# NVlabs/few-shot-vid2vid

Hardware: AMD Instinct MI355X
Metric: frames/sec G+D fwd+bwd step, 512x512 fewshot_pose (higher is better)
Workload: dtype f32; 1 GPU; fewshot_pose 512x512, per-GPU batch 2, adaptive_spade+warp_ref+spade_combine, D step + G step (train.py:58-62), Adam included, no VGG / no FlowNet2 / face-D; global_batch=2, parallelism=dp1, launch=hipgraph

## Files before the change

few-shot-vid2vid_amd/conv.py:

```python
import ctypes
import os
import threading

import torch

from . import lib, profile

ACT_NONE, ACT_LRELU, ACT_TANH, ACT_SIGMOID, ACT_RELU, ACT_LRELU01, ACT_DLRELU = (
    lib.ENUMS["FSV_ACT_" + k] for k in ("NONE", "LRELU", "TANH", "SIGMOID", "RELU", "LRELU01", "DLRELU"))

MFMA_F32, MFMA_F16, MFMA_BF16X3 = 0, 1, 2
_MFMA_NAMES = {'': 0, '0': 0, 'f32': 0, 'fp32': 0, '1': 1, 'f16': 1, 'fp16': 1, '2': 2, 'bf16x3': 2}
_mfma_mode = _MFMA_NAMES[os.environ.get('FSV_MFMA_MODE', '').lower()]


def set_mfma_mode(mode):
    global _mfma_mode
    prev = _mfma_mode
    _mfma_mode = _MFMA_NAMES[str(mode).lower()] if not isinstance(mode, int) else int(mode)
    if _mfma_mode not in (0, 1, 2):
        _mfma_mode = prev
        raise ValueError("unknown MFMA operand mode %r" % (mode,))
    return prev

# ... 368 lines not shown
        if ns > 1 and act != ACT_DLRELU:
            split_ws = torch.empty(ns * out.numel(), dtype=torch.float32, device=x.device)
    ws_args = (lib.ptr(split_ws), split_ws.numel() if split_ws is not None else 0)
    if entry == "fsv_conv_gather_fwd_np":
        if up:
            raise ValueError("a folded up-sampling needs the exact-fp32 kernels (conv.up_foldable)")
        args = head + (_np_mode, lib.stream_ptr())
    else:
        args = head + ws_args + (1 if up else 0, lib.stream_ptr())
    if (stats is not None and grp is None and entry == "fsv_conv_gather_fwd" and place is None and not per_sample
            and not accumulate and force_tile < 0 and force_split == 0 and cin % 4 == 0 and stats_enabled()):
        groups = int(stats['groups'])
        part = stats_arena(x.device).take(groups * STATS_SLOTS * cout * 2)
        prezeroed = part is not None
        if part is None:
            part = torch.empty(groups * STATS_SLOTS * cout * 2, dtype=torch.float64, device=x.device)
        produced = ctypes.c_int(0)
        sargs = (lib.ptr(x), lib.ptr(wt), lib.ptr(bias), lib.ptr(res), lib.ptr(out), n, h, w, cin, oh, ow, cout, len(ty),
                 lib.int_array(ty), lib.int_array(tx), sy, sx, ldw, act, float(scale), lib.ptr(wscale), lib.ptr(part), groups,
                 STATS_SLOTS, 1 if prezeroed else 0, ctypes.byref(produced)) + ws_args + (1 if up else 0, lib.stream_ptr())
        label = 'fsv_conv_igemm_kernel'
        if profile.enabled():
            label = profile.conv_label(n * oh * ow, cout, (len(ty) * cin + 31) // 32, 1, True, force_tile, force_split)
        keep = (x, wt, bias, res, out, wscale, part, split_ws)

        def go_stats(sargs=sargs, keep=keep):
            lib.call("fsv_conv_gather_fwd_stats", *sargs)
        with profile.scope(label, 2.0 * n * oh * ow * cout * cin * len(ty), replay=go_stats):
            go_stats()
        if produced.value:
            stats['part'], stats['slots'] = part, STATS_SLOTS
        return out
    if grp is not None and entry == "fsv_conv_gather_fwd" and force_tile < 0 and force_split == 0:
        d = ConvDesc()
        d.inp, d.wt, d.bias, d.res, d.out, d.wscale = (t.data_ptr() if t is not None else None
                                                       for t in (x, wt, bias, res, out, wscale))
        d.N, d.H, d.W, d.Cin, d.OH, d.OW, d.Cout, d.ntaps = n, h, w, cin, oh, ow, cout, len(ty)
        for i, (a, b) in enumerate(zip(ty, tx)):
            d.ty[i], d.tx[i] = a, b
        d.sy, d.sx, d.outH, d.outW, d.osy, d.osx, d.ooy, d.oox, d.ldw = sy, sx, out_h, out_w, osy, osx, ooy, oox, ldw
        d.per_sample, d.act, d.accumulate, d.scale = (1 if per_sample else 0), act, (1 if accumulate else 0), float(scale)
        d.w_bstride, d.b_bstride = w_bs, b_bs
        label = 'fsv_conv_igemm_kernel'
        if profile.enabled():
            label = profile.conv_label(oh * ow if per_sample else n * oh * ow, cout, (len(ty) * cin + 31) // 32,
                                       n if per_sample else 1, cin % 4 == 0, force_tile, force_split)
        grp.convs.append((d, entry, args, label, 2.0 * n * oh * ow * cout * cin * len(ty), (x, wt, bias, res, out, wscale)))
        return out
    if profile.enabled():
        mz = oh * ow if per_sample else n * oh * ow
        label = profile.conv_label(mz, cout, (len(ty) * cin + 31) // 32, n if per_sample else 1, cin % 4 == 0,
                                   force_tile, force_split,
                                   thin=0 if entry.endswith('_np') else _thin_k(cout, cin, len(ty), per_sample, place, accumulate,
                                                                                force_tile, force_split, act))
        if entry.endswith('_np'):
            label = label.replace('fsv_conv_igemm_kernel', 'fsv_np_conv_kernel[%s]' % ('f16' if _np_mode == 1 else 'bf16x3'))
        keep = (x, wt, bias, res, out, wscale, split_ws)

        def go(entry=entry, args=args, keep=keep):
            lib.call(entry, *args)
        with profile.scope(label, 2.0 * n * oh * ow * cout * cin * len(ty), replay=go):
            go()
    else:
        lib.call(entry, *args)
    return out


_tickets = {}
_TICKET_POOL = 1 << 16


def ticket_range(like, n):
    n = (max(int(n), 1) + 63) // 64 * 64
    if n > _TICKET_POOL // 4:
        return None
    ent = _tickets.get(like.device)
    if ent is None:
        from . import streams
        ent = _tickets[like.device] = [streams.shared(lambda: torch.zeros(_TICKET_POOL, dtype=torch.int32, device=like.device)), 0]
    pool, cur = ent
    if cur + n > _TICKET_POOL:
        cur = 0
    ent[1] = (cur + n) % _TICKET_POOL
    return ctypes.c_void_p(pool.data_ptr() + 4 * cur)


def ordered_split():
    return os.environ.get('FSV_ORDERED_SPLIT', '1') == '1'


def _thin_k(cout, cin, ntaps, per_sample, place, accumulate, force_tile, force_split, act):
    q = cin >> 2
    ok = (cout <= 4 and cin % 4 == 0 and cin <= 256 and q & (q - 1) == 0 and ntaps * cin <= 1152 and not per_sample and
          place is None and not accumulate and force_tile < 0 and force_split <= 0 and act != ACT_DLRELU)
    return ntaps * cin if ok else 0


def conv_forward(x, wt_f, ldw, cout, geom, bias=None, res=None, act=ACT_NONE, scale=1.0, per_sample=False,
                 force_tile=-1, force_split=0, wscale=None, stats=None, up=False):
    n, cin, h, w = x.shape
    oh, ow = geom.out_hw(2 * h, 2 * w) if up else geom.out_hw(h, w)
    return gather_gemm(x, wt_f, ldw, cout, oh, ow, geom.ty, geom.tx, geom.stride, geom.stride, bias=bias, res=res,
                       act=act, scale=scale, per_sample=per_sample, force_tile=force_tile, force_split=force_split,
                       wscale=wscale, stats=stats, up=up)


def planned(mz, cout, nchunks, nsamp, force_tile=-1, force_split=0):
    tile, nsplit = ctypes.c_int(0), ctypes.c_int(1)
    lib.call("fsv_conv_plan", mz, cout, nchunks, nsamp, force_tile, force_split, ctypes.byref(tile), ctypes.byref(nsplit))
    return tile.value, nsplit.value


def _planned_split(mz, cout, nchunks, nsamp):
    return planned(mz, cout, nchunks, nsamp)[1]


_plan_log = None


def start_plan_log():
    global _plan_log
    _plan_log = []


def stop_plan_log():
    global _plan_log
    log, _plan_log = _plan_log, None
    return log or []


def conv_dgrad(dout, w, geom, in_hw, scale=None, per_sample=False, cached=None, cin=None, out_half=False):
    dout = to_nhwc(dout)
    n, cout, oh, ow = dout.shape
    cin = w.shape[-3] if cin is None else cin
    h, wd = in_hw
    s = geom.stride
    if dout.dtype == torch.float16:
        from . import hconv
        layouts = []
        for k, c in enumerate(geom.dgrad_classes):
            if not c['khs']:
                layouts.append(None)
            elif cached is not None:
                layouts.append(half_twin(cached[k][0]))
            else:
                wt_k, _, _ = prep_weight(w, 1, geom, c['khs'], c['kws'], None)
                layouts.append(half_twin(wt_k))
        return hconv.conv_dgrad_h(dout, layouts, geom, in_hw, cin, scale=scale, per_sample=per_sample, out_half=out_half)
# ... 22 lines not shown
            mz = sh * sw if per_sample else n * sh * sw
            if _planned_split(mz, cin, (len(c['khs']) * cout + 31) // 32, n if per_sample else 1) > 1:
                plain = False
                break
    dx = empty_nhwc(n, cin, h, wd, dout) if plain else zeros_nhwc(n, cin, h, wd, dout)
    with launch_group(grouped):
        for k, (c, (sub_h, sub_w)) in enumerate(zip(geom.dgrad_classes, subs)):
            if sub_h <= 0 or sub_w <= 0 or not c['khs']:
                continue
            wt, ldw, ws = layout(k, c)
            gather_gemm(dout, wt, ldw, cin, sub_h, sub_w, c['ty'], c['tx'], 1, 1, per_sample=per_sample, out=dx,
                        place=(h, wd, s, s, c['py'], c['px']), accumulate=not plain, wscale=ws)
    return dx


def conv_wgrad(x, dout, geom, w_shape, per_sample=False, scale=None, force_split=0, out=None, raw=False, arena=None,
               force_tile=0, up=False):
    x = to_nhwc(x)
    dout = to_nhwc(dout)
    n, cin, h, w = x.shape
    if up:
        if x.dtype != torch.float32 or dout.dtype != torch.float32 or per_sample or narrow_staging_mode():
            raise ValueError("a folded up-sampling needs the exact-fp32 kernels (conv.up_foldable)")
        h, w = 2 * h, 2 * w
    _, cout, oh, ow = dout.shape
    if x.dtype == torch.float16 or dout.dtype == torch.float16:
        from . import hconv
        if hconv.wgrad_eligible(cin, cout, oh, ow) and force_tile == 0:
            dwt = hconv.conv_wgrad_h(hconv.to_half_nhwc(x), hconv.to_half_nhwc(dout), geom, per_sample=per_sample,
                                     force_split=force_split, arena=arena if raw else None)
            if raw:
                return dwt
            return unprep_weight_grad(dwt, tuple(w_shape), geom, scale, out)
        x, dout = hconv.cast(x, torch.float32), hconv.cast(dout, torch.float32)
    kpad = _ceil(geom.ntaps * cin, 32)
    ldw = _ceil(cout, 32)
    nb = n if per_sample else 1
    dwt = arena.take(kpad * ldw) if (arena is not None and raw and not per_sample) else None
    prezeroed = dwt is not None
    if dwt is None:
        dwt = torch.empty((nb, kpad, ldw), dtype=torch.float32, device=x.device)
    lib.check_device(x, dout)
    kdim, vec4 = geom.ntaps * cin, cin % 4 == 0
    bn = 32 if cout <= 32 else (64 if cout <= 64 else 128)
    bm = 128
    if vec4 and bn >= 64:
        bm = 32 if kdim <= 32 else (64 if kdim <= 64 else 128)
    if force_tile == 0 and vec4 and cout >= 64 and kdim > 64 and os.environ.get('FSV_WGRAD_PLAN', '1') == '1':
        bm, bn = 64, 64
    label = 'fsv_conv_wgrad_kernel<%dx%d,V%d>' % (bm, bn, 4 if vec4 else 1)
    if (profile.enabled() and cout <= 4 and vec4 and not per_sample and force_tile == 0 and force_split <= 0 and
            geom.ntaps * (cin >> 2) <= 256 and not narrow_staging_mode() and profile.thin_rule(n * oh * ow, kdim)):
        label = 'fsv_conv_thin_wgrad_kernel<Cout%d>' % cout
    if profile.detail():
        label += ' Kdim%d N%d pix%d z%d' % (geom.ntaps * cin, cout, (oh * ow) if per_sample else n * oh * ow, nb)
    _np_mode = narrow_staging_mode()
    narrow = _np_mode and vec4
    if narrow:
        label = 'fsv_np_wgrad_kernel[%s]' % ('f16' if _np_mode == 1 else 'bf16x3')
    wargs = (lib.ptr(x), lib.ptr(dout), lib.ptr(dwt), n, h, w, cin, oh, ow, cout,
             geom.ntaps, lib.int_array(geom.ty), lib.int_array(geom.tx), geom.stride, geom.stride,
             ldw, kpad, kpad * ldw, 1 if per_sample else 0, force_split, 1 if prezeroed else 0, force_tile)
    grp = _active_group()
    if (grp is not None and not narrow and prezeroed and raw and vec4 and force_split == 0 and force_tile == 0
            and 32 // ow + 1 <= oh and not up):
        d = WgradDesc()
        d.inp, d.dout, d.dwt = x.data_ptr(), dout.data_ptr(), dwt.data_ptr()
        d.N, d.H, d.W, d.Cin, d.OH, d.OW, d.Cout, d.ntaps = n, h, w, cin, oh, ow, cout, geom.ntaps
        for i, (a, b) in enumerate(zip(geom.ty, geom.tx)):
            d.ty[i], d.tx[i] = a, b
        d.sy, d.sx, d.ldw, d.Kpad, d.per_sample, d.reserved, d.w_bstride = geom.stride, geom.stride, ldw, kpad, 0, 0, kpad * ldw
        grp.wgrads.append((d, "fsv_conv_wgrad", wargs + (0, lib.stream_ptr()), label,
                           2.0 * n * oh * ow * cout * cin * geom.ntaps, (x, dout, dwt)))
        return dwt
    with profile.scope(label, 2.0 * n * oh * ow * cout * cin * geom.ntaps):
        if narrow:
            lib.call("fsv_conv_wgrad_np", *wargs, _np_mode, lib.stream_ptr())
        else:
            lib.call("fsv_conv_wgrad", *wargs, 1 if up else 0, lib.stream_ptr())
    if raw:
        return dwt
    return unprep_weight_grad(dwt, tuple(w_shape), geom, scale, out)
```

few-shot-vid2vid_amd/csrc/conv_igemm.hip:

```cpp
#include <stdlib.h>
#include "conv_igemm.h"


__device__ __forceinline__ void fsv_xcd_tile(int nx, int ny, int& bx, int& by) {
  const int b = blockIdx.x + blockIdx.y * nx;
  if ((nx & 7) != 0 || ny == 1) { bx = blockIdx.x; by = blockIdx.y; return; }
  const int xcd = b & 7, j = b >> 3;
  by = j % ny;
  bx = xcd + 8 * (j / ny);
}

template <int BM, int BN, int WM, int WN, int PF, bool AF, int DBG = 0, int MODE = 0, bool UP = false>
__device__ __forceinline__ void fsv_conv_igemm_body(const ConvP& p, const int bx, const int by, const int bz) {
  constexpr bool LD = MODE == 2, WT = MODE >= 1;
  constexpr int BK = FSV_BK;
  constexpr int NT = 64 * WM * WN;
  constexpr int RPA = NT / 8;
  constexpr int TM = BM / (WM * 32), TN = BN / (WN * 32);
  constexpr int NPA = BM / RPA;
  constexpr int QB = BN / 4;
  constexpr int RPB = NT / QB;
  constexpr int NPB = BK / RPB;
  constexpr int A_ST = BM * BK, B_ST = BK * BN;
  static_assert(TM >= 1 && TN >= 1 && NPA >= 1 && NPA * RPA == BM && NPB >= 1 && NPB * RPB == BK, "tile / thread-count mismatch");
// ... 1137 lines not shown
  {
    unsigned long long code = (t < 8) ? p.taps_lo : p.taps_hi;
    int sh = (t & 7) * 8;
    ty = (int)((code >> sh) & 15ull) - 8;
    tx = (int)((code >> (sh + 4)) & 15ull) - 8;
  }
  const fsv_buf abuf = fsv_make_buf(p.in, (long long)p.N * p.H * p.W * p.Cin * 4);
  const fsv_buf dbuf = fsv_make_buf(p.dout, (long long)p.Mz * p.Cout * 4);
  const int ohw = p.OH * p.OW;
  const int m0 = blockIdx.x * chunk;
  const int m1 = (m0 + chunk < p.Mz) ? m0 + chunk : p.Mz;
  float acc[4][CO];
#pragma unroll
  for (int e = 0; e < 4; ++e)
#pragma unroll
    for (int c = 0; c < CO; ++c) acc[e][c] = 0.f;
  if (lane_on) {
#pragma unroll 4
    for (int m = m0 + g; m < m1; m += NG) {
      const int n = m / ohw, rem = m - n * ohw;
      const int oy = rem / p.OW, ox = rem - oy * p.OW;
      const int iy = oy * p.sy + ty, ix = ox * p.sx + tx;
      const bool ok = ((unsigned)iy < (unsigned)p.H) & ((unsigned)ix < (unsigned)p.W);
      const float4 v = fsv_buf_load4(abuf, ok ? (unsigned)((((n * p.H + iy) * p.W + ix) * p.Cin + ci) * 4) : FSV_BUF_OOB);
      float d[CO];
#pragma unroll
      for (int c = 0; c < CO; ++c) d[c] = fsv_buf_load1(dbuf, (c < p.Cout) ? (unsigned)((m * p.Cout + c) * 4) : FSV_BUF_OOB);
#pragma unroll
      for (int c = 0; c < CO; ++c) {
        acc[0][c] = fmaf(v.x, d[c], acc[0][c]);
        acc[1][c] = fmaf(v.y, d[c], acc[1][c]);
        acc[2][c] = fmaf(v.z, d[c], acc[2][c]);
        acc[3][c] = fmaf(v.w, d[c], acc[3][c]);
      }
    }
  }
#pragma unroll
  for (int e = 0; e < 4; ++e)
#pragma unroll
    for (int c = 0; c < CO; ++c) red[(e * CO + c) * 256 + tid] = acc[e][c];
  __syncthreads();
  if (g == 0) {
#pragma unroll
    for (int e = 0; e < 4; ++e)
#pragma unroll
      for (int c = 0; c < CO; ++c) {
        float s = 0.f;
        for (int gg = 0; gg < NG; ++gg) s += red[(e * CO + c) * 256 + gg * QK + q];
        if (c < p.Cout) atomicAdd(p.dwt + (long long)(t * p.Cin + ci + e) * p.ldw + c, s);
      }
  }
}

static inline bool fsv_conv_thin(int Mz, int K) {
  const int sw = (int)fsv_env("FSV_CONV_THIN", 1);
  if (sw == 0) return false;
  if (sw == 2) return true;
  return K <= 1152 && (long long)Mz >= 64ll * K;
}

__global__ __launch_bounds__(256) void fsv_prep_weight_kernel(const float* w, float* wt, const float* scale_ptr,
                                                              int mode_in, int Cout, int Cin, int KH, int KW,
                                                              int ntaps, unsigned long long taps_lo,
                                                              unsigned long long taps_hi, int Kpad, int ldw,
                                                              long long w_bstride, long long wt_bstride) {
  const int z = blockIdx.z;
  const float s = scale_ptr ? *scale_ptr : 1.f;
  const long long total = (long long)Kpad * ldw;
  const bool accum = mode_in == 3;
  const int mode = accum ? 2 : mode_in;
  const int rowlen = (mode == 1) ? Cout : Cin;
  const int ncols = (mode == 1) ? Cin : Cout;
  const int K = ntaps * rowlen;
  long long i = (long long)blockIdx.x * 256 + threadIdx.x;
  const long long stride = (long long)gridDim.x * 256;
  for (; i < total; i += stride) {
    int r = (int)(i / ldw), c = (int)(i - (long long)r * ldw);
    bool ok = r < K && c < ncols;
    int j = ok ? r / rowlen : 0;
    int a = r - j * rowlen;
    unsigned long long code = (j < 8) ? taps_lo : taps_hi;
    int sh = (j & 7) * 8;
    int kh = (int)((code >> sh) & 15ull), kw = (int)((code >> (sh + 4)) & 15ull);
    int co = (mode == 1) ? a : c, ci = (mode == 1) ? c : a;
    long long widx = (((long long)co * Cin + ci) * KH + kh) * KW + kw + (long long)z * w_bstride;
    if (mode == 2) {
      if (ok) {
        float g = s * wt[(long long)z * wt_bstride + i];
        ((float*)w)[widx] = accum ? ((float*)w)[widx] + g : g;
      }
    } else {
      wt[(long long)z * wt_bstride + i] = ok ? s * w[widx] : 0.f;
    }
  }
}

struct PrepGroup {
  const long long* src; const long long* dst; const int* dims; const unsigned long long* taps;
};
template <int KKT>
__device__ __forceinline__ void fsv_prep_stage(const PrepGroup& g, const int layer, const int cot, const int cit, float* t) {
  const int* d = g.dims + layer * 9;
  const int Cout = d[0], CinR = d[2], KW = d[4];
  const int KK = KKT ? KKT : d[3] * KW;
  const int CI_T = KK <= 8 ? 32 : 16;
  const int run = CI_T * KK, lds = run + 1;
  const float* w = reinterpret_cast<const float*>(g.src[layer]);
  const int co0 = cot * 32, ci0 = cit * CI_T;
  const int tid = threadIdx.x;
  const int total = 32 * run;
  constexpr int U = 8;
// ... 309 lines not shown
  p.in = in; p.wt = wt; p.bias = bias; p.res = res; p.out = out; p.wscale = wscale;
  p.N = N; p.H = H; p.W = W; p.Cin = Cin; p.OH = OH; p.OW = OW; p.Cout = Cout;
  p.K = ntaps * Cin; p.nchunks = fsv_cdiv(p.K, FSV_BK); p.ldw = ldw;
  p.sy = sy; p.sx = sx; p.ntaps = ntaps;
  fsv_pack_taps(ty, tx, ntaps, p.taps_lo, p.taps_hi, 8);
  p.outH = outH; p.outW = outW; p.osy = osy; p.osx = osx; p.ooy = ooy; p.oox = oox;
  p.dense_out = (osy == 1 && osx == 1 && ooy == 0 && oox == 0 && outH == OH && outW == OW) ? 1 : 0;
  p.w_bstride = w_bstride; p.b_bstride = b_bstride; p.per_sample = per_sample ? 1 : 0;
  p.act = act; p.scale = scale;
  p.Mz = per_sample ? OH * OW : N * OH * OW;
  p.nsplit = 1;
  p.stats = nullptr; p.stats_slots = 1; p.stats_ohw = 1;
  p.part = nullptr; p.part_stride = 0;
  p.up = 0;
  {
    const long long obytes = (long long)N * outH * outW * Cout * 4;
    p.res_bytes = (res && obytes <= FSV_BUF_MAX_BYTES) ? obytes : 0;
  }
}

static inline bool vec4_ok(int cin) { return (cin & 3) == 0; }

static inline int fsv_conv_check_args(const float* in, const float* wt, const float* out, int N, int H, int W, int Cin, int Cout,
                                      int ntaps, const int* ty, const int* tx, int ldw) {
  if (!in || !wt || !out || ntaps < 1 || ntaps > 16 || N < 1 || Cin < 1 || Cout < 1) return FSV_ERR_BAD_ARG;
  for (int t = 0; t < ntaps; ++t)
    if (ty[t] < -8 || ty[t] > 7 || tx[t] < -8 || tx[t] > 7) return FSV_ERR_UNSUPPORTED;
  if ((ldw & 3) != 0 || ldw < Cout) return FSV_ERR_BAD_ARG;
  if ((long long)N * H * W * Cin * 4 > FSV_BUF_MAX_BYTES || (long long)(ntaps * Cin + 32) * ldw * 4 > FSV_BUF_MAX_BYTES) return FSV_ERR_UNSUPPORTED;
  return FSV_OK;
}

static int fsv_conv_gather_impl(const float* in, const float* wt, const float* bias, const float* res, float* out,
                        int N, int H, int W, int Cin, int OH, int OW, int Cout,
                        int ntaps, const int* ty, const int* tx, int sy, int sx,
                        int outH, int outW, int osy, int osx, int ooy, int oox,
                        int ldw, long long w_bstride, long long b_bstride, int per_sample,
                        int act, float scale, int force_tile, int force_split, int accumulate, const float* wscale,
                        double* stats, int stats_groups, int stats_slots, int stats_prezeroed, int* produced,
                        float* split_ws, long long split_cap, int in_up, hipStream_t stream) {
  if (const int bad = fsv_conv_check_args(in, wt, out, N, H, W, Cin, Cout, ntaps, ty, tx, ldw)) return bad;
  if (in_up && ((H & 1) || (W & 1) || (Cin % 4 != 0) || per_sample || accumulate || Cout <= 4)) return FSV_ERR_UNSUPPORTED;
  ConvP p;
  fsv_fill_convp(p, in, wt, bias, res, out, wscale, N, H, W, Cin, OH, OW, Cout, ntaps, ty, tx, sy, sx, outH, outW, osy, osx, ooy,
                 oox, ldw, w_bstride, b_bstride, per_sample, act, scale);
  p.up = in_up ? 1 : 0;
  const int nsamp = per_sample ? N : 1;
  int tile = 0, nsplit = 1;
  if (Cout <= 4 && (Cin % 4 == 0) && Cin <= 256 && ((Cin >> 2) & ((Cin >> 2) - 1)) == 0 && p.K <= FSV_THIN_MAXK && !per_sample &&
      p.dense_out && !accumulate && force_tile < 0 && force_split <= 0 && !stats &&
      act != FSV_ACT_DLRELU && fsv_conv_thin(p.Mz, p.K)) {
    p.nsplit = 1;
    if (produced) *produced = 0;
    const int ppb = 4 * (64 / (Cin >> 2));
    int iters = 16;
    while (iters > 1 && fsv_cdiv(p.Mz, ppb * iters) < 1024) iters >>= 1;
    const dim3 g(fsv_cdiv(p.Mz, ppb * iters));
    switch (Cout) {
      case 1: FSV_LAUNCH((fsv_conv_thin_fwd_kernel<1>), g, dim3(256), stream, p, iters); break;
      case 2: FSV_LAUNCH((fsv_conv_thin_fwd_kernel<2>), g, dim3(256), stream, p, iters); break;
      case 3: FSV_LAUNCH((fsv_conv_thin_fwd_kernel<3>), g, dim3(256), stream, p, iters); break;
      default: FSV_LAUNCH((fsv_conv_thin_fwd_kernel<4>), g, dim3(256), stream, p, iters); break;
    }
    return fsv_check_launch();
  }
  if (act == FSV_ACT_DLRELU) {
    if (!res || accumulate) return FSV_ERR_BAD_ARG;
    force_split = 1;
  }
  if (fsv_conv_plan(p.Mz, Cout, p.nchunks, nsamp, force_tile, force_split, &tile, &nsplit)) return FSV_ERR_BAD_ARG;
  p.nsplit = nsplit;
  const long long total = (long long)N * outH * outW * Cout;
  if (accumulate) {
    if (bias || res || act != FSV_ACT_NONE || scale != 1.f) return FSV_ERR_BAD_ARG;
  } else if (nsplit > 1) {
    if (!p.dense_out) return FSV_ERR_UNSUPPORTED;
    if (split_ws && (Cin % 4 == 0) && split_cap >= (long long)nsplit * total) {
      p.part = split_ws; p.part_stride = total;
    } else {
      (void)hipMemsetAsync(out, 0, (size_t)total * sizeof(float), stream);
    }
  }
  const bool vec4 = (Cin % 4 == 0);
  if (produced) *produced = 0;
  if (stats && vec4 && nsplit == 1 && !accumulate && !per_sample && p.dense_out && stats_groups >= 1 && stats_slots >= 1 &&
      p.Mz % stats_groups == 0 && (stats_groups == 1 || p.Mz / stats_groups >= 128)) {
    p.stats = stats; p.stats_slots = stats_slots; p.stats_ohw = p.Mz / stats_groups;
    if (!stats_prezeroed)
      (void)hipMemsetAsync(stats, 0, (size_t)stats_groups * stats_slots * Cout * 2 * sizeof(double), stream);
    if (produced) *produced = 1;
  }
  double* fin_stats = nullptr;
  {
    if (stats && fsv_env("FSV_SPLIT_FIN_STATS", 1) != 0 && fsv_env("FSV_SPLIT_FIN4", 1) != 0 && nsplit > 1 && p.part && !accumulate && !per_sample && p.dense_out &&
        stats_groups >= 1 && stats_slots >= 1 && (Cout % 32) == 0 && p.Mz % stats_groups == 0 && ((p.Mz / stats_groups) % 32) == 0 &&
        act != FSV_ACT_DLRELU && !fsv_deterministic() &&
        (((unsigned long long)p.part | (unsigned long long)out | (unsigned long long)res) & 15ull) == 0) {
      fin_stats = stats;
      if (!stats_prezeroed)
        (void)hipMemsetAsync(stats, 0, (size_t)stats_groups * stats_slots * Cout * 2 * sizeof(double), stream);
      if (produced) *produced = 1;
    }
  }
  if (force_tile < 0 && vec4) tile = fsv_conv_variant(tile);
  int rc = fsv_launch_conv(p, vec4, nsamp * nsplit, stream, tile);
  if (rc) return rc;
  if (!accumulate && nsplit > 1 && (p.part || bias || res || act != FSV_ACT_NONE || scale != 1.f)) {
    int grid = (int)((total + 256 * 8 - 1) / (256 * 8));
    if (grid > 4096) grid = 4096;
    if (grid < 1) grid = 1;
    const bool fin4 = fsv_env("FSV_SPLIT_FIN4", 1) != 0 && p.part && (Cout % 4 == 0) && (total % 4 == 0) &&
                      (((unsigned long long)p.part | (unsigned long long)out | (unsigned long long)res) & 15ull) == 0;
    if (fin_stats) {
      const long long npix = (long long)N * outH * outW;
      FSV_LAUNCH(fsv_split_finish4_stats_kernel, dim3((unsigned)((npix + 31) / 32), (unsigned)(Cout / 32)), dim3(256), stream,
                 (const float4*)p.part, p.part_stride / 4, nsplit, (float4*)out, bias, (const float4*)res, npix, Cout, act, scale,
// ... 35 lines not shown
                              double* stats, int stats_groups, int stats_slots, int stats_prezeroed, int* produced,
                              float* split_ws, long long split_ws_floats, int in_up, hipStream_t stream) {
  if (!stats || !produced) return FSV_ERR_BAD_ARG;
  return fsv_conv_gather_impl(in, wt, bias, res, out, N, H, W, Cin, OH, OW, Cout, ntaps, ty, tx, sy, sx, OH, OW, 1, 1, 0, 0, ldw,
                              0, 0, 0, act, scale, -1, 0, 0, wscale, stats, stats_groups, stats_slots, stats_prezeroed, produced,
                              split_ws, split_ws ? split_ws_floats : 0, in_up, stream);
}

int fsv_bias_act(float* x, const float* bias, long long total, int C, int act, hipStream_t stream) {
  if (!x || total < 1 || C < 1) return FSV_ERR_BAD_ARG;
  int grid = (int)((total + 256 * 8 - 1) / (256 * 8));
  if (grid > 4096) grid = 4096;
  if (grid < 1) grid = 1;
  FSV_LAUNCH(fsv_bias_act_kernel, dim3(grid), dim3(256), stream, x, bias, (const float*)nullptr, total, C, 1ll, 0ll, act,
             1.f);
  return fsv_check_launch();
}

}

static inline void fsv_fill_wgradp(WgradP& p, const float* in, const float* dout, float* dwt, int N, int H, int W, int Cin, int OH,
                                   int OW, int Cout, int ntaps, const int* ty, const int* tx, int sy, int sx, int ldw,
                                   long long w_bstride, int per_sample, int in_up) {
  p.in = in; p.dout = dout; p.dwt = dwt;
  p.N = N; p.H = H; p.W = W; p.Cin = Cin; p.OH = OH; p.OW = OW; p.Cout = Cout;
  p.K = ntaps * Cin; p.ldw = ldw; p.sy = sy; p.sx = sx; p.ntaps = ntaps;
  fsv_pack_taps(ty, tx, ntaps, p.taps_lo, p.taps_hi, 8);
  p.w_bstride = w_bstride; p.per_sample = per_sample ? 1 : 0;
  p.Mz = per_sample ? OH * OW : N * OH * OW;
  p.pchunks = fsv_cdiv(p.Mz, FSV_BK);
  p.up = in_up ? 1 : 0;
}

extern "C" {

int fsv_conv_wgrad(const float* in, const float* dout, float* dwt,
                   int N, int H, int W, int Cin, int OH, int OW, int Cout,
                   int ntaps, const int* ty, const int* tx, int sy, int sx,
                   int ldw, int Kpad, long long w_bstride, int per_sample, int force_split, int prezeroed,
                   int force_tile, int in_up, hipStream_t stream) {
  if (!in || !dout || !dwt || ntaps < 1 || ntaps > 16) return FSV_ERR_BAD_ARG;
  if (in_up && ((H & 1) || (W & 1) || (Cin % 4 != 0) || (Cout & 3) != 0 || Cout <= 4 || per_sample || FSV_BK / OW + 1 > OH))
    return FSV_ERR_UNSUPPORTED;
  for (int t = 0; t < ntaps; ++t)
    if (ty[t] < -8 || ty[t] > 7 || tx[t] < -8 || tx[t] > 7) return FSV_ERR_UNSUPPORTED;
  if ((long long)N * H * W * Cin * 4 > FSV_BUF_MAX_BYTES || (long long)N * OH * OW * Cout * 4 > FSV_BUF_MAX_BYTES) return FSV_ERR_UNSUPPORTED;
  WgradP p;
  fsv_fill_wgradp(p, in, dout, dwt, N, H, W, Cin, OH, OW, Cout, ntaps, ty, tx, sy, sx, ldw, w_bstride, per_sample, in_up);
  const int nsamp = per_sample ? N : 1;
  if (Cout <= 4 && vec4_ok(Cin) && !per_sample && force_tile == 0 && force_split <= 0 && ntaps * (Cin >> 2) <= 256 &&
      fsv_conv_thin(p.Mz, p.K)) {
    p.nsplit = 1;
    if (!prezeroed) (void)hipMemsetAsync(dwt, 0, (size_t)Kpad * ldw * sizeof(float), stream);
    int chunk = fsv_cdiv(p.Mz, 512);
    if (chunk < 64) chunk = 64;
    const dim3 g(fsv_cdiv(p.Mz, chunk));
    switch (Cout) {
      case 1: FSV_LAUNCH((fsv_conv_thin_wgrad_kernel<1>), g, dim3(256), stream, p, chunk); break;
      case 2: FSV_LAUNCH((fsv_conv_thin_wgrad_kernel<2>), g, dim3(256), stream, p, chunk); break;
      case 3: FSV_LAUNCH((fsv_conv_thin_wgrad_kernel<3>), g, dim3(256), stream, p, chunk); break;
      default: FSV_LAUNCH((fsv_conv_thin_wgrad_kernel<4>), g, dim3(256), stream, p, chunk); break;
    }
    return fsv_check_launch();
  }
  int bn = (Cout <= 32) ? 32 : (Cout <= 64 ? 64 : 128);
  int bmk = 128;
  if (vec4_ok(Cin) && bn >= 64) bmk = (p.K <= 32) ? 32 : (p.K <= 64 ? 64 : 128);
  if (force_tile == 1 && vec4_ok(Cin) && Cout > 32) { bmk = 64; bn = 64; }
  else if (force_tile == 2 && vec4_ok(Cin) && Cout > 32) { bmk = 128; bn = 64; }
  else if (force_tile == 3 && vec4_ok(Cin) && Cout > 64) { bmk = 64; bn = 128; }
  else if (force_tile == 4 && vec4_ok(Cin) && Cout > 64) { bmk = 128; bn = 128; }
  long long target = fsv_tune(2);
  static int wplan_v = -1;
  if (wplan_v < 0) wplan_v = (int)fsv_env("FSV_WGRAD_PLAN", 1);
  if (force_tile == 0 && wplan_v == 1 && vec4_ok(Cin) && Cout >= 64 && p.K > 64) {
    bmk = 64; bn = 64; target = 2048;
  }
  long long blocks = (long long)fsv_cdiv(p.K, bmk) * fsv_cdiv(Cout, bn) * nsamp;
  int nsplit = 1;
  if (force_split > 0) nsplit = force_split;
  else if (fsv_deterministic()) nsplit = 1;
  else {
    nsplit = (int)((target + blocks - 1) / blocks);
    int maxs = p.pchunks / (int)fsv_tune(3);
    if (nsplit > maxs) nsplit = maxs;
    if (nsplit < 1) nsplit = 1;
  }
  if (nsplit > p.pchunks) nsplit = p.pchunks;
  p.nsplit = nsplit;
  if (nsplit > 1 && !prezeroed)
    (void)hipMemsetAsync(dwt, 0, (size_t)((per_sample ? (long long)N * w_bstride : (long long)Kpad * ldw)) * sizeof(float), stream);
  dim3 block(256);
  const bool vec4 = (Cin % 4 == 0) && (FSV_BK / OW + 1 <= OH) && ((Cout & 3) == 0 || bn == 32);
  dim3 g(fsv_cdiv(p.K, bmk), fsv_cdiv(Cout, bn), nsamp * nsplit);
  if (vec4) {
    if (bn == 128 && bmk == 32) FSV_LAUNCH((fsv_conv_wgrad_kernel<32, 128, 1, 4, true>), g, block, stream, p);
    else if (bn == 128 && bmk == 64) FSV_LAUNCH((fsv_conv_wgrad_kernel<64, 128, 2, 2, true>), g, block, stream, p);
    else if (bn == 64 && bmk == 32) FSV_LAUNCH((fsv_conv_wgrad_kernel<32, 64, 1, 2, true>), g, dim3(128), stream, p);
    else if (bn == 64 && bmk == 64) FSV_LAUNCH((fsv_conv_wgrad_kernel<64, 64, 2, 2, true>), g, block, stream, p);
    else if (bn == 128) FSV_LAUNCH((fsv_conv_wgrad_kernel<128, 128, 2, 2, true>), g, block, stream, p);
    else if (bn == 64) FSV_LAUNCH((fsv_conv_wgrad_kernel<128, 64, 2, 2, true>), g, block, stream, p);
    else if ((Cout & 3) == 0) FSV_LAUNCH((fsv_conv_wgrad_kernel<128, 32, 4, 1, true>), g, block, stream, p);
    else FSV_LAUNCH((fsv_conv_wgrad_kernel<128, 32, 4, 1, false>), g, block, stream, p);
  } else {
    if (bn == 128) FSV_LAUNCH((fsv_conv_wgrad_v1_kernel<128, 128, 2, 2>), g, block, stream, p);
    else if (bn == 64) FSV_LAUNCH((fsv_conv_wgrad_v1_kernel<128, 64, 2, 2>), g, block, stream, p);
// ... 201 lines not shown
```

few-shot-vid2vid_amd/profile.py:

```python
import ctypes

import torch

from . import lib

_enabled = False
_only = None
_detail = False
_records = []
FP32_MFMA_PEAK = 157.3e12
F16_MFMA_PEAK = 2.5e15

_tiles = None


def tile_table():
    global _tiles
    if _tiles is None:
        out = (ctypes.c_int * 6)()
        _tiles = {i: tuple(out) for i in range(64) if lib.call_status("fsv_conv_tile_info", i, out) == 0}
    return _tiles


def tile_name(tile):
# ... 45 lines not shown
def stamp_result(st):
    torch.cuda.synchronize()
    n = st['n']
    if n == 0:
        return 0, 0.0, 0.0
    khz = int(lib.get_lib().fsv_stamp_rate_khz())
    if khz <= 0:
        return 0, 0.0, 0.0
    t = st['buf'][:4 * n].cpu().view(n, 4).double()
    full = (t[:, 1] - t[:, 0]).mean().item() / (khz * 1e3)
    empty = (t[:, 3] - t[:, 2]).mean().item() / (khz * 1e3)
    return n, full, empty


class scope:
    def __init__(self, label, flops, replay=None):
        self.label, self.flops, self.replay = label, flops, replay

    def __enter__(self):
        self.on = _enabled and _events and not lib.is_emu() and (_only is None or self.label == _only)
        self.st = _stamp if (_stamp is not None and self.label == _stamp['label'] and _stamp['n'] < _stamp['cap']) else None
        if self.st is not None:
            k = 4 * self.st['n']
            lib.call("fsv_stamp", _stamp_slot(self.st, k + 2), lib.stream_ptr())
            lib.call("fsv_stamp", _stamp_slot(self.st, k + 3), lib.stream_ptr())
            lib.call("fsv_stamp", _stamp_slot(self.st, k), lib.stream_ptr())
        if self.on:
            self.e0 = torch.cuda.Event(enable_timing=True)
            self.e1 = torch.cuda.Event(enable_timing=True)
            self.e0.record()
        return self

    def __exit__(self, *exc):
        if self.on:
            self.e1.record()
            _records.append((self.label, self.flops, self.e0, self.e1, None if _only is not None else self.replay))
        if self.st is not None:
            lib.call("fsv_stamp", _stamp_slot(self.st, 4 * self.st['n'] + 1), lib.stream_ptr())
            self.st['n'] += 1
        return False


def bracket_average(label):
    torch.cuda.synchronize()
    ts = [e0.elapsed_time(e1) * 1e-3 for lab, _, e0, e1, _ in _records if lab == label]
    _records.clear()
    return len(ts), (sum(ts) / len(ts) if ts else 0.0)


def thin_rule(mz, k):
    return lib.call_status("fsv_conv_thin_rule", int(mz), int(k)) == 1


def conv_label(mz, cout, nchunks, nsamp, vec4, force_tile=-1, force_split=0, thin=0):
    if thin and thin_rule(mz, thin):
        base = 'fsv_conv_thin_fwd_kernel<Cout%d>' % cout
        if _detail:
            base += ' M%d N%d K%d' % (mz, cout, nchunks * 32)
        return base
    tile, nsplit = ctypes.c_int(0), ctypes.c_int(1)
    lib.call("fsv_conv_plan", mz, cout, nchunks, nsamp, force_tile, force_split, ctypes.byref(tile), ctypes.byref(nsplit))
    base = 'fsv_conv_igemm_kernel<%s,V%d>' % (tile_name(tile.value), 4 if vec4 else 1)
    if _detail:
        base += ' M%d N%d K%d z%d split%d' % (mz, cout, nchunks * 32, nsamp, nsplit.value)
    return base


def summary():
    torch.cuda.synchronize()
    agg = {}
    for label, flops, e0, e1, _ in _records:
        a = agg.setdefault(label, [0, 0.0, 0.0])
        a[0] += 1
        a[1] += flops
        a[2] += e0.elapsed_time(e1) * 1e-3
    by_kernel = {}
    for label, (n, fl, t) in agg.items():
        by_kernel[label] = dict(launches=n, avg_us=round(t / n * 1e6, 2), total_ms=round(t * 1e3, 3),
                                tflops=round(fl / t / 1e12, 2) if t > 0 else 0.0,
                                gflop_per_launch=round(fl / n / 1e9, 3))
    dominant = None
    if agg:
        lab = max(agg, key=lambda k: agg[k][2])
        n, fl, t = agg[lab]
        ach = fl / t / 1e12
        peak = FP32_MFMA_PEAK / 1e12
        if '[f16]' in lab or lab.startswith('fsv_hconv'):
            peak = F16_MFMA_PEAK / 1e12
        elif '[bf16x3]' in lab:
            peak = F16_MFMA_PEAK / 3e12
        bracketed = t / n
        replays = [r[4] for r in _records if r[0] == lab and r[4] is not None]
        replay_us = None
        if len(replays) == n:
            reps = 3
            for r in replays:
                r()
            e0, e1 = torch.cuda.Event(enable_timing=True), torch.cuda.Event(enable_timing=True)
            e0.record()
            for _ in range(reps):
                for r in replays:
                    r()
            e1.record()
            torch.cuda.synchronize()
            replay_us = e0.elapsed_time(e1) * 1e3 / reps / n
        dominant = dict(kernel=lab, bound='mfma', achieved=round(ach, 2), peak=round(peak, 1), unit='TFLOP/s',
                        frac=round(ach / peak, 4), traffic=None, launches=n,
                        avg_launch_us=round(bracketed * 1e6, 2), bracketed_us=round(bracketed * 1e6, 2),
                        replay_us_warm_cache_upper_bound=None if replay_us is None else round(replay_us, 2),
# ... 8 lines not shown
```

Before: 47.12 frames/s.

## Add shared-memory spatial tile kernels for thin-channel 3x3 convs fwd/wgrad/dgrad

Adds three new kernels for convolutions with very few channels on one side and 3x3-or-smaller stride-1 taps: a tiled forward kernel and a tiled weight-gradient kernel for Cout<=4, plus a thin kernel for Cin<=4 with Cout up to 64 (e.g. the data-gradient or first-layer case). Each stages a haloed 32-wide spatial tile in LDS so neighbouring taps reuse loaded pixels instead of re-gathering per tap through the MFMA implicit-GEMM path. This targets the memory-bound thin convs where the GEMM tiles are mostly padding. It adds many template instantiations, atomics in the wgrad reduction, and new dispatch conditions gated by FSV_THIN_TILE.

```diff
diff --git a/few-shot-vid2vid_amd/conv.py b/few-shot-vid2vid_amd/conv.py
--- a/few-shot-vid2vid_amd/conv.py
+++ b/few-shot-vid2vid_amd/conv.py
@@ -444,14 +444,18 @@
         label = profile.conv_label(mz, cout, (len(ty) * cin + 31) // 32, n if per_sample else 1, cin % 4 == 0,
                                    force_tile, force_split,
                                    thin=0 if entry.endswith('_np') else _thin_k(cout, cin, len(ty), per_sample, place, accumulate,
-                                                                                force_tile, force_split, act))
+                                                                                force_tile, force_split, act),
+                                   tile=thin_tile_geom(cin, ty, tx, sy, sx),
+                                   thin_dgrad=0 if (entry.endswith('_np') or up) else _thin_dgrad_k(
+                                       cout, cin, ty, tx, sy, sx, per_sample, place, accumulate, force_tile, force_split, act))
         if entry.endswith('_np'):
             label = label.replace('fsv_conv_igemm_kernel', 'fsv_np_conv_kernel[%s]' % ('f16' if _np_mode == 1 else 'bf16x3'))
         keep = (x, wt, bias, res, out, wscale, split_ws)
 
         def go(entry=entry, args=args, keep=keep):
             lib.call(entry, *args)
-        with profile.scope(label, 2.0 * n * oh * ow * cout * cin * len(ty), replay=go):
+        mfma_flop = 0.0 if label.startswith('fsv_conv_thin_dgrad_kernel') else 2.0 * n * oh * ow * cout * cin * len(ty)
+        with profile.scope(label, mfma_flop, replay=go):
             go()
     else:
         lib.call(entry, *args)
@@ -486,6 +490,21 @@
     ok = (cout <= 4 and cin % 4 == 0 and cin <= 256 and q & (q - 1) == 0 and ntaps * cin <= 1152 and not per_sample and
           place is None and not accumulate and force_tile < 0 and force_split <= 0 and act != ACT_DLRELU)
     return ntaps * cin if ok else 0
+
+
+def thin_tile_taps(ty, tx, sy, sx):
+    return (sy == 1 and sx == 1 and all(-1 <= a <= 1 for a in ty) and all(-1 <= b <= 1 for b in tx) and
+            float(os.environ.get('FSV_THIN_TILE', '1') or 0) != 0)
+
+
+def thin_tile_geom(cin, ty, tx, sy, sx):
+    return cin in (8, 16, 32, 64) and len(ty) * cin <= 576 and thin_tile_taps(ty, tx, sy, sx)
+
+
+def _thin_dgrad_k(cout, cin, ty, tx, sy, sx, per_sample, place, accumulate, force_tile, force_split, act):
+    ok = (cin <= 4 and cout in (8, 16, 32, 64) and len(ty) in (1, 9) and not per_sample and place is None and not accumulate and
+          force_tile < 0 and force_split <= 0 and act != ACT_DLRELU and thin_tile_taps(ty, tx, sy, sx))
+    return len(ty) * cin if ok else 0
 
 
 def conv_forward(x, wt_f, ldw, cout, geom, bias=None, res=None, act=ACT_NONE, scale=1.0, per_sample=False,
@@ -614,6 +633,8 @@
     if (profile.enabled() and cout <= 4 and vec4 and not per_sample and force_tile == 0 and force_split <= 0 and
             geom.ntaps * (cin >> 2) <= 256 and not narrow_staging_mode() and profile.thin_rule(n * oh * ow, kdim)):
         label = 'fsv_conv_thin_wgrad_kernel<Cout%d>' % cout
+        if not up and thin_tile_geom(cin, geom.ty, geom.tx, geom.stride, geom.stride):
+            label = 'fsv_conv_thin_tile_wgrad_kernel<Cout%d>' % cout
     if profile.detail():
         label += ' Kdim%d N%d pix%d z%d' % (geom.ntaps * cin, cout, (oh * ow) if per_sample else n * oh * ow, nb)
     _np_mode = narrow_staging_mode()
diff --git a/few-shot-vid2vid_amd/csrc/conv_igemm.hip b/few-shot-vid2vid_amd/csrc/conv_igemm.hip
--- a/few-shot-vid2vid_amd/csrc/conv_igemm.hip
+++ b/few-shot-vid2vid_amd/csrc/conv_igemm.hip
@@ -1213,11 +1213,326 @@
   }
 }
 
+#define FSV_TT_W 32
+#define FSV_TT_PITCH 35
+#define FSV_TT_FLOATS (FSV_TT_PITCH * 10 * 32)
+#define FSV_TT_MAXK 576
+static inline int fsv_tt_rows(int Cin) { return Cin == 64 ? 3 : (Cin == 32 ? 8 : (Cin == 16 ? 16 : 32)); }
+
+__device__ __forceinline__ void fsv_tt_stage(float* tile, const fsv_buf& abuf, int n, int y0, int x0, int th, int H, int W, int Cin,
+                                             int qshift, int tid) {
+  const int rowq = (FSV_TT_W + 2) << qshift;
+  const int total = (th + 2) * rowq;
+#pragma unroll 1
+  for (int i0 = tid; i0 < total; i0 += 6 * 256) {
+    float4 v[6];
+    int dst[6];
+#pragma unroll
+    for (int u = 0; u < 6; ++u) {
+      const int i = i0 + u * 256;
+      const int r = i / rowq, c = i - r * rowq;
+      const int px = c >> qshift;
+      const int iy = y0 - 1 + r, ix = x0 - 1 + px;
+      const bool ok = (i < total) & ((unsigned)iy < (unsigned)H) & ((unsigned)ix < (unsigned)W);
+      v[u] = fsv_buf_load4(abuf, ok ? (unsigned)((((n * H + iy) * W + ix) * Cin) * 4 + ((c - (px << qshift)) << 4)) : FSV_BUF_OOB);
+      dst[u] = (i < total) ? r * FSV_TT_PITCH * Cin + c * 4 : -1;
+    }
+#pragma unroll
+    for (int u = 0; u < 6; ++u)
+      if (dst[u] >= 0) *(float4*)(tile + dst[u]) = v[u];
+  }
+}
+
+template <int CO, int NT>
+__global__ __launch_bounds__(256) void fsv_conv_thin_tile_fwd_kernel(ConvP p, int th, int iters) {
+  __shared__ float wl[FSV_TT_MAXK * CO];
+  __shared__ __attribute__((aligned(16))) float tile[FSV_TT_FLOATS];
+  const int tid = threadIdx.x, lane = tid & 63, wave = tid >> 6;
+  for (int i = tid; i < p.K * CO; i += 256) {
+    const int k = i / CO, c = i - k * CO;
+    wl[i] = (c < p.Cout) ? p.wt[(long long)k * p.ldw + c] : 0.f;
+  }
+  const int QC = p.Cin >> 2;
+  const int qshift = 31 - __builtin_clz(QC);
+  const int PPW = 64 / QC;
+  const int cq = lane % QC, pl = lane / QC;
+  float wr[NT > 0 ? NT * 4 * CO : 1];
+  int toff[NT > 0 ? NT : 1];
+  if (NT > 0) {
+    __syncthreads();
+#pragma unroll
+    for (int t = 0; t < NT; ++t) {
+#pragma unroll
+      for (int e = 0; e < 4 * CO; ++e) wr[t * 4 * CO + e] = wl[(t * p.Cin + cq * 4) * CO + e];
+      int ty, tx;
+      fsv_tap(p, t, ty, tx);
+      toff[t] = (ty * FSV_TT_PITCH + tx) * p.Cin;
+    }
+  }
+  const fsv_buf abuf = fsv_make_buf(p.in, (long long)p.N * p.H * p.W * p.Cin * 4);
+  const float ws = p.wscale ? p.wscale[0] : 1.f;
+  const int tiles_x = (p.OW + FSV_TT_W - 1) / FSV_TT_W, tiles_y = (p.OH + th - 1) / th;
+  const int ntiles = p.N * tiles_y * tiles_x;
+  const int ngroups = th * FSV_TT_W / PPW;
+#pragma unroll 1
+  for (int it = 0; it < iters; ++it) {
+    const int tix = blockIdx.x * iters + it;
+    if (tix >= ntiles) break;
+    const int n = tix / (tiles_y * tiles_x), trem = tix - n * (tiles_y * tiles_x);
+    const int y0 = (trem / tiles_x) * th, x0 = (trem % tiles_x) * FSV_TT_W;
+    fsv_tt_stage(tile, abuf, n, y0, x0, th, p.H, p.W, p.Cin, qshift, tid);
+    __syncthreads();
+#pragma unroll 1
+    for (int g = wave; g < ngroups; g += 4) {
+      const int pi = g * PPW + pl;
+      const int ly = pi >> 5, lx = pi & 31;
+      const int oy = y0 + ly, ox = x0 + lx;
+      const bool live = (oy < p.OH) & (ox < p.OW);
+      const float* t0 = tile + ((ly + 1) * FSV_TT_PITCH + lx + 1) * p.Cin + cq * 4;
+      float acc[CO];
+#pragma unroll
+      for (int c = 0; c < CO; ++c) acc[c] = 0.f;
+      if (NT > 0) {
+#pragma unroll
+        for (int t = 0; t < NT; ++t) {
+          const float4 v = *(const float4*)(t0 + toff[t]);
+          const float* w0 = wr + t * 4 * CO;
+#pragma unroll
+          for (int c = 0; c < CO; ++c) {
+            acc[c] = fmaf(v.x, w0[c], acc[c]);
+            acc[c] = fmaf(v.y, w0[CO + c], acc[c]);
+            acc[c] = fmaf(v.z, w0[2 * CO + c], acc[c]);
+            acc[c] = fmaf(v.w, w0[3 * CO + c], acc[c]);
+          }
+        }
+      } else {
+#pragma unroll 3
+        for (int t = 0; t < p.ntaps; ++t) {
+          int ty, tx;
+          fsv_tap(p, t, ty, tx);
+          const float4 v = *(const float4*)(t0 + (ty * FSV_TT_PITCH + tx) * p.Cin);
+          const float* w0 = wl + (t * p.Cin + cq * 4) * CO;
+#pragma unroll
+          for (int c = 0; c < CO; ++c) {
+            acc[c] = fmaf(v.x, w0[c], acc[c]);
+            acc[c] = fmaf(v.y, w0[CO + c], acc[c]);
+            acc[c] = fmaf(v.z, w0[2 * CO + c], acc[c]);
+            acc[c] = fmaf(v.w, w0[3 * CO + c], acc[c]);
+          }
+        }
+      }
+      for (int o = 1; o < QC; o <<= 1) {
+#pragma unroll
+        for (int c = 0; c < CO; ++c) acc[c] += __shfl_xor(acc[c], o);
+      }
+      const long long m = ((long long)n * p.OH + oy) * p.OW + ox;
+      if (QC >= 4) {
+        float a = acc[0];
+#pragma unroll
+        for (int c = 1; c < CO; ++c) a = (cq == c) ? acc[c] : a;
+        if (live && cq < p.Cout) {
+          float v = a * ws;
+          v = (v + (p.bias ? p.bias[cq] : 0.f)) * p.scale;
+          v = fsv_act(v, p.act);
+          if (p.res) v += p.res[m * p.Cout + cq];
+          p.out[m * p.Cout + cq] = v;
+        }
+      } else if (live && cq == 0) {
+#pragma unroll
+        for (int c = 0; c < CO; ++c) {
+          if (c >= p.Cout) break;
+          float v = acc[c] * ws;
+          v = (v + (p.bias ? p.bias[c] : 0.f)) * p.scale;
+          v = fsv_act(v, p.act);
+          if (p.res) v += p.res[m * p.Cout + c];
+          p.out[m * p.Cout + c] = v;
+        }
+      }
+    }
+    __syncthreads();
+  }
+}
+
+template <int CO>
+__global__ __launch_bounds__(256) void fsv_conv_thin_tile_wgrad_kernel(WgradP p, int th, int iters) {
+  __shared__ __attribute__((aligned(16))) float tile[FSV_TT_FLOATS];
+  __shared__ __attribute__((aligned(16))) float dl[FSV_TT_W * 8 * CO];
+  const int QC = p.Cin >> 2;
+  const int qshift = 31 - __builtin_clz(QC);
+  const int QK = p.ntaps * QC;
+  const int NG = 256 / QK;
+  const int tid = threadIdx.x;
+  const int q = tid % QK, g = tid / QK;
+  const bool lane_on = g < NG;
+  const int t = q / QC, ci = (q - t * QC) * 4;
+  int ty, tx;
+  {
+    unsigned long long code = (t < 8) ? p.taps_lo : p.taps_hi;
+    int sh = (t & 7) * 8;
+    ty = (int)((code >> sh) & 15ull) - 8;
+    tx = (int)((code >> (sh + 4)) & 15ull) - 8;
+  }
+  const fsv_buf abuf = fsv_make_buf(p.in, (long long)p.N * p.H * p.W * p.Cin * 4);
+  const fsv_buf dbuf = fsv_make_buf(p.dout, (long long)p.Mz * p.Cout * 4);
+  const int tiles_x = (p.OW + FSV_TT_W - 1) / FSV_TT_W, tiles_y = (p.OH + th - 1) / th;
+  const int ntiles = p.N * tiles_y * tiles_x;
+  const int npix = th * FSV_TT_W;
+  const float* t0 = tile + ((1 + ty) * FSV_TT_PITCH + 1 + tx) * p.Cin + ci;
+  float acc[4][CO];
+#pragma unroll
+  for (int e = 0; e < 4; ++e)
+#pragma unroll
+    for (int c = 0; c < CO; ++c) acc[e][c] = 0.f;
+#pragma unroll 1
+  for (int it = 0; it < iters; ++it) {
+    const int tix = blockIdx.x * iters + it;
+    if (tix >= ntiles) break;
+    const int n = tix / (tiles_y * tiles_x), trem = tix - n * (tiles_y * tiles_x);
+    const int y0 = (trem / tiles_x) * th, x0 = (trem % tiles_x) * FSV_TT_W;
+    fsv_tt_stage(tile, abuf, n, y0, x0, th, p.H, p.W, p.Cin, qshift, tid);
+    for (int i = tid; i < npix * CO; i += 256) {
+      const int pi = i / CO, c = i - pi * CO;
+      const int oy = y0 + (pi >> 5), ox = x0 + (pi & 31);
+      const bool ok = (oy < p.OH) & (ox < p.OW) & (c < p.Cout);
+      dl[i] = fsv_buf_load1(dbuf, ok ? (unsigned)(((((n * p.OH + oy) * p.OW + ox) * p.Cout) + c) * 4) : FSV_BUF_OOB);
+    }
+    __syncthreads();
+    if (lane_on) {
+      const int nlive = ((p.OH - y0 < th) ? p.OH - y0 : th) * FSV_TT_W;
+#pragma unroll 4
+      for (int pi = g; pi < nlive; pi += NG) {
+        const int ly = pi >> 5, lx = pi & 31;
+        const float4 v = *(const float4*)(t0 + (ly * FSV_TT_PITCH + lx) * p.Cin);
+        float d[CO];
+#pragma unroll
+        for (int c = 0; c < CO; ++c) d[c] = dl[pi * CO + c];
+#pragma unroll
+        for (int c = 0; c < CO; ++c) {
+          acc[0][c] = fmaf(v.x, d[c], acc[0][c]);
+          acc[1][c] = fmaf(v.y, d[c], acc[1][c]);
+          acc[2][c] = fmaf(v.z, d[c], acc[2][c]);
+          acc[3][c] = fmaf(v.w, d[c], acc[3][c]);
+        }
+      }
+    }
+    __syncthreads();
+  }
+  float* red = tile;
+#pragma unroll
+  for (int e = 0; e < 4; ++e)
+#pragma unroll
+    for (int c = 0; c < CO; ++c) red[(e * CO + c) * 256 + tid] = acc[e][c];
+  __syncthreads();
+  if (g == 0) {
+#pragma unroll
+    for (int e = 0; e < 4; ++e)
+#pragma unroll
+      for (int c = 0; c < CO; ++c) {
+        float s = 0.f;
+        for (int gg = 0; gg < NG; ++gg) s += red[(e * CO + c) * 256 + gg * QK + q];
+        if (c < p.Cout) atomicAdd(p.dwt + (long long)(t * p.Cin + ci + e) * p.ldw + c, s);
+      }
+  }
+}
+
+#define FSV_TD_ROWS 16
+template <int CI, int NT>
+__global__ __launch_bounds__(256) void fsv_conv_thin_dgrad_kernel(ConvP p, int iters) {
+  __shared__ float4 dl[(FSV_TD_ROWS + 2) * (FSV_TT_W + 2)];
+  const int tid = threadIdx.x, lane = tid & 63, wave = tid >> 6;
+  const int QC = p.Cout >> 2;
+  const int PPW = 64 / QC;
+  const int cq = lane % QC, pl = lane / QC;
+  float4 w[NT * CI];
+#pragma unroll
+  for (int k = 0; k < NT * CI; ++k) w[k] = *(const float4*)(p.wt + (long long)k * p.ldw + cq * 4);
+  int toff[NT];
+#pragma unroll
+  for (int t = 0; t < NT; ++t) {
+    int ty, tx;
+    fsv_tap(p, t, ty, tx);
+    toff[t] = ty * (FSV_TT_W + 2) + tx;
+  }
+  const fsv_buf abuf = fsv_make_buf(p.in, (long long)p.N * p.H * p.W * CI * 4);
+  const float ws = p.wscale ? p.wscale[0] : 1.f;
+  float4 bv = make_float4(0.f, 0.f, 0.f, 0.f);
+  if (p.bias) bv = make_float4(p.bias[cq * 4], p.bias[cq * 4 + 1], p.bias[cq * 4 + 2], p.bias[cq * 4 + 3]);
+  const int tiles_x = (p.OW + FSV_TT_W - 1) / FSV_TT_W, tiles_y = (p.OH + FSV_TD_ROWS - 1) / FSV_TD_ROWS;
+  const int ntiles = p.N * tiles_y * tiles_x;
+  const int ngroups = FSV_TD_ROWS * FSV_TT_W / PPW;
+#pragma unroll 1
+  for (int it = 0; it < iters; ++it) {
+    const int tix = blockIdx.x * iters + it;
+    if (tix >= ntiles) break;
+    const int n = tix / (tiles_y * tiles_x), trem = tix - n * (tiles_y * tiles_x);
+    const int y0 = (trem / tiles_x) * FSV_TD_ROWS, x0 = (trem % tiles_x) * FSV_TT_W;
+    for (int i = tid; i < (FSV_TD_ROWS + 2) * (FSV_TT_W + 2); i += 256) {
+      const int r = i / (FSV_TT_W + 2), c = i - r * (FSV_TT_W + 2);
+      const int iy = y0 - 1 + r, ix = x0 - 1 + c;
+      const bool ok = ((unsigned)iy < (unsigned)p.H) & ((unsigned)ix < (unsigned)p.W);
+      const unsigned off = ok ? (unsigned)((((n * p.H + iy) * p.W + ix) * CI) * 4) : FSV_BUF_OOB;
+      float4 v = make_float4(0.f, 0.f, 0.f, 0.f);
+      v.x = fsv_buf_load1(abuf, off);
+      if (CI > 1) v.y = fsv_buf_load1(abuf, ok ? off + 4 : FSV_BUF_OOB);
+      if (CI > 2) v.z = fsv_buf_load1(abuf, ok ? off + 8 : FSV_BUF_OOB);
+      if (CI > 3) v.w = fsv_buf_load1(abuf, ok ? off + 12 : FSV_BUF_OOB);
+      dl[i] = v;
+    }
+    __syncthreads();
+#pragma unroll 1
+    for (int g = wave; g < ngroups; g += 4) {
+      const int pi = g * PPW + pl;
+      const int ly = pi >> 5, lx = pi & 31;
+      const int oy = y0 + ly, ox = x0 + lx;
+      const float4* d0 = dl + (ly + 1) * (FSV_TT_W + 2) + lx + 1;
+      float4 acc = make_float4(0.f, 0.f, 0.f, 0.f);
+#pragma unroll
+      for (int t = 0; t < NT; ++t) {
+        const float4 d = d0[toff[t]];
+#pragma unroll
+        for (int c = 0; c < CI; ++c) {
+          const float dc = (c == 0) ? d.x : (c == 1 ? d.y : (c == 2 ? d.z : d.w));
+          const float4 wk = w[t * CI + c];
+          acc.x = fmaf(dc, wk.x, acc.x);
+          acc.y = fmaf(dc, wk.y, acc.y);
+          acc.z = fmaf(dc, wk.z, acc.z);
+          acc.w = fmaf(dc, wk.w, acc.w);
+        }
+      }
+      if ((oy < p.OH) & (ox < p.OW)) {
+        const long long m = ((long long)n * p.OH + oy) * p.OW + ox;
+        float4 v;
+        v.x = fsv_act((acc.x * ws + bv.x) * p.scale, p.act);
+        v.y = fsv_act((acc.y * ws + bv.y) * p.scale, p.act);
+        v.z = fsv_act((acc.z * ws + bv.z) * p.scale, p.act);
+        v.w = fsv_act((acc.w * ws + bv.w) * p.scale, p.act);
+        if (p.res) {
+          const float4 r = *(const float4*)(p.res + m * p.Cout + cq * 4);
+          v.x += r.x; v.y += r.y; v.z += r.z; v.w += r.w;
+        }
+        *(float4*)(p.out + m * p.Cout + cq * 4) = v;
+      }
+    }
+    __syncthreads();
+  }
+}
+
 static inline bool fsv_conv_thin(int Mz, int K) {
   const int sw = (int)fsv_env("FSV_CONV_THIN", 1);
   if (sw == 0) return false;
   if (sw == 2) return true;
   return K <= 1152 && (long long)Mz >= 64ll * K;
+}
+
+static inline bool fsv_thin_tile_taps(int ntaps, const int* ty, const int* tx, int sy, int sx) {
+  if (sy != 1 || sx != 1) return false;
+  for (int t = 0; t < ntaps; ++t)
+    if (ty[t] < -1 || ty[t] > 1 || tx[t] < -1 || tx[t] > 1) return false;
+  return true;
+}
+static inline bool fsv_thin_tile_geom(int Cin, int ntaps, const int* ty, const int* tx, int sy, int sx) {
+  if (Cin != 8 && Cin != 16 && Cin != 32 && Cin != 64) return false;
+  return fsv_thin_tile_taps(ntaps, ty, tx, sy, sx) && fsv_env("FSV_THIN_TILE", 1) != 0;
 }
 
 __global__ __launch_bounds__(256) void fsv_prep_weight_kernel(const float* w, float* wt, const float* scale_ptr,
@@ -1633,6 +1948,28 @@
       act != FSV_ACT_DLRELU && fsv_conv_thin(p.Mz, p.K)) {
     p.nsplit = 1;
     if (produced) *produced = 0;
+    if (fsv_thin_tile_geom(Cin, ntaps, ty, tx, sy, sx) && p.K <= FSV_TT_MAXK) {
+      const int th = fsv_tt_rows(Cin);
+      const int ntiles = N * fsv_cdiv(OH, th) * fsv_cdiv(OW, FSV_TT_W);
+      int iters = fsv_cdiv(ntiles, 768);
+      if (iters < 2) iters = 2;
+      const dim3 g(fsv_cdiv(ntiles, iters));
+      switch (Cout) {
+        case 1: if (ntaps == 9) FSV_LAUNCH((fsv_conv_thin_tile_fwd_kernel<1, 9>), g, dim3(256), stream, p, th, iters);
+                else FSV_LAUNCH((fsv_conv_thin_tile_fwd_kernel<1, 0>), g, dim3(256), stream, p, th, iters);
+                break;
+        case 2: if (ntaps == 9) FSV_LAUNCH((fsv_conv_thin_tile_fwd_kernel<2, 9>), g, dim3(256), stream, p, th, iters);
+                else FSV_LAUNCH((fsv_conv_thin_tile_fwd_kernel<2, 0>), g, dim3(256), stream, p, th, iters);
+                break;
+        case 3: if (ntaps == 9) FSV_LAUNCH((fsv_conv_thin_tile_fwd_kernel<3, 9>), g, dim3(256), stream, p, th, iters);
+                else FSV_LAUNCH((fsv_conv_thin_tile_fwd_kernel<3, 0>), g, dim3(256), stream, p, th, iters);
+                break;
+        default: if (ntaps == 9) FSV_LAUNCH((fsv_conv_thin_tile_fwd_kernel<4, 9>), g, dim3(256), stream, p, th, iters);
+                else FSV_LAUNCH((fsv_conv_thin_tile_fwd_kernel<4, 0>), g, dim3(256), stream, p, th, iters);
+                break;
+      }
+      return fsv_check_launch();
+    }
     const int ppb = 4 * (64 / (Cin >> 2));
     int iters = 16;
     while (iters > 1 && fsv_cdiv(p.Mz, ppb * iters) < 1024) iters >>= 1;
@@ -1643,6 +1980,25 @@
       case 3: FSV_LAUNCH((fsv_conv_thin_fwd_kernel<3>), g, dim3(256), stream, p, iters); break;
       default: FSV_LAUNCH((fsv_conv_thin_fwd_kernel<4>), g, dim3(256), stream, p, iters); break;
     }
+    return fsv_check_launch();
+  }
+  if (Cin <= 4 && (Cout == 8 || Cout == 16 || Cout == 32 || Cout == 64) && (ntaps == 1 || ntaps == 9) && !per_sample && p.dense_out &&
+      !accumulate && force_tile < 0 && force_split <= 0 && !stats && !in_up && act != FSV_ACT_DLRELU &&
+      fsv_thin_tile_taps(ntaps, ty, tx, sy, sx) && fsv_env("FSV_THIN_TILE", 1) != 0 && fsv_conv_thin(p.Mz, p.K) &&
+      (((unsigned long long)wt | (unsigned long long)out | (unsigned long long)res) & 15ull) == 0) {
+    p.nsplit = 1;
+    if (produced) *produced = 0;
+    const int ntiles = N * fsv_cdiv(OH, FSV_TD_ROWS) * fsv_cdiv(OW, FSV_TT_W);
+    int iters = 8;
+    while (iters > 2 && fsv_cdiv(ntiles, iters) < 1024) iters >>= 1;
+    const dim3 g(fsv_cdiv(ntiles, iters));
+#define FSV_TD_CASE(ci, nt) \
+    case ci * 16 + nt: FSV_LAUNCH((fsv_conv_thin_dgrad_kernel<ci, nt>), g, dim3(256), stream, p, iters); break;
+    switch (Cin * 16 + ntaps) {
+      FSV_TD_CASE(1, 1) FSV_TD_CASE(2, 1) FSV_TD_CASE(3, 1) FSV_TD_CASE(4, 1)
+      FSV_TD_CASE(1, 9) FSV_TD_CASE(2, 9) FSV_TD_CASE(3, 9) FSV_TD_CASE(4, 9)
+    }
+#undef FSV_TD_CASE
     return fsv_check_launch();
   }
   if (act == FSV_ACT_DLRELU) {
@@ -1784,6 +2140,19 @@
       fsv_conv_thin(p.Mz, p.K)) {
     p.nsplit = 1;
     if (!prezeroed) (void)hipMemsetAsync(dwt, 0, (size_t)Kpad * ldw * sizeof(float), stream);
+    if (!in_up && fsv_thin_tile_geom(Cin, ntaps, ty, tx, sy, sx) && p.K <= FSV_TT_MAXK) {
+      const int th = fsv_tt_rows(Cin) < 8 ? fsv_tt_rows(Cin) : 8;
+      const int ntiles = N * fsv_cdiv(OH, th) * fsv_cdiv(OW, FSV_TT_W);
+      const int iters = ntiles > 768 ? fsv_cdiv(ntiles, 768) : 4;
+      const dim3 g(fsv_cdiv(ntiles, iters));
+      switch (Cout) {
+        case 1: FSV_LAUNCH((fsv_conv_thin_tile_wgrad_kernel<1>), g, dim3(256), stream, p, th, iters); break;
+        case 2: FSV_LAUNCH((fsv_conv_thin_tile_wgrad_kernel<2>), g, dim3(256), stream, p, th, iters); break;
+        case 3: FSV_LAUNCH((fsv_conv_thin_tile_wgrad_kernel<3>), g, dim3(256), stream, p, th, iters); break;
+        default: FSV_LAUNCH((fsv_conv_thin_tile_wgrad_kernel<4>), g, dim3(256), stream, p, th, iters); break;
+      }
+      return fsv_check_launch();
+    }
     int chunk = fsv_cdiv(p.Mz, 512);
     if (chunk < 64) chunk = 64;
     const dim3 g(fsv_cdiv(p.Mz, chunk));
diff --git a/few-shot-vid2vid_amd/profile.py b/few-shot-vid2vid_amd/profile.py
--- a/few-shot-vid2vid_amd/profile.py
+++ b/few-shot-vid2vid_amd/profile.py
@@ -121,9 +121,14 @@
     return lib.call_status("fsv_conv_thin_rule", int(mz), int(k)) == 1
 
 
-def conv_label(mz, cout, nchunks, nsamp, vec4, force_tile=-1, force_split=0, thin=0):
+def conv_label(mz, cout, nchunks, nsamp, vec4, force_tile=-1, force_split=0, thin=0, tile=False, thin_dgrad=0):
+    if thin_dgrad and thin_rule(mz, thin_dgrad):
+        base = 'fsv_conv_thin_dgrad_kernel<Cin%d>' % (thin_dgrad if thin_dgrad <= 4 else thin_dgrad // 9)
+        if _detail:
+            base += ' M%d N%d K%d' % (mz, cout, nchunks * 32)
+        return base
     if thin and thin_rule(mz, thin):
-        base = 'fsv_conv_thin_fwd_kernel<Cout%d>' % cout
+        base = ('fsv_conv_thin_tile_fwd_kernel<Cout%d>' if tile else 'fsv_conv_thin_fwd_kernel<Cout%d>') % cout
         if _detail:
             base += ' M%d N%d K%d' % (mz, cout, nchunks * 32)
         return base
```

Measured after the change: 47.53 frames/s, median of 6. Within noise of the previous version (+0.9%).
